# rohitsinghlab/SAME

Measured on AMD Instinct MI355X. Metric: cell-pairs/sec on 100k×100k cost build + edge-cross sweep; % HBM roofline, higher is better.
Workload: dtype f64

## Files before the change

### include/same_hip_diag.h

```cpp
#ifndef SAME_HIP_DIAG_H
#define SAME_HIP_DIAG_H

#include "same_hip.h"

#ifdef __cplusplus
extern "C" {
#endif

enum { SAME_STAT_LAUNCHES = 0, SAME_STAT_FILLS = 1, SAME_STAT_COPIES = 2, SAME_STAT_WAITS = 3, SAME_STAT_GREEDY_READBACKS = 4, SAME_STAT_COUNT = 5 };
int same_ctx_stat(same_ctx *ctx, int which, int64_t *out);


int same_timer_start(same_ctx *ctx);
int same_timer_stop(same_ctx *ctx, float *out_ms);
int same_timer_mark(same_ctx *ctx);
int same_timer_read(same_ctx *ctx, float *out_ms);

int same_ctx_pci_bus_id(same_ctx *ctx, char *out, size_t out_len);
int same_dev_mem_info(same_ctx *ctx, int64_t *out_free, int64_t *out_total);

#define SAME_SPREAD_INFO_LEN 14
int same_dev_alloc_spread(same_ctx *ctx, size_t bytes, void **out_dptr, int64_t *out_info);

#define SAME_Q32_MAX_TYPES 32
int same_quantize_u32_dev(same_ctx *ctx, const double *dsrc, int64_t n, double offset, double scale,
                          uint32_t *ddst);
int same_dense_cost_q32_dev(same_ctx *ctx, const uint32_t *dAq, const uint32_t *dRq, const double *dA,
                            const double *dR, int T, const double *daxy, const double *drxy, int64_t n_r,
                            int64_t row_begin, int64_t row_end, double w, double inv_scale,
                            double rel_tol, double *dout, int64_t ld);

int same_comm_gather_time(same_ctx *ctx, float *out_ms, int64_t *out_send_bytes);

#ifdef __cplusplus
}
#endif
#endif
```

### same_amd/_lib.py

```python
import ctypes
import os
import sys
import threading

import numpy as np

_HERE = os.path.dirname(os.path.abspath(__file__))
LIB_PATH = os.environ.get("SAME_HIP_LIB") or os.path.join(_HERE, "libsame_hip.so")

c_i64 = ctypes.c_int64
c_int = ctypes.c_int
c_dbl = ctypes.c_double
c_flt = ctypes.c_float
c_vp = ctypes.c_void_p
c_sz = ctypes.c_size_t

UNIQUE_ID_BYTES = 128
ABI_VERSION = 8
DT_U8, DT_I32, DT_U64, DT_F64 = 0, 1, 2, 3
OP_SUM, OP_MAX, OP_MIN = 0, 1, 2
SPREAD_INFO_LEN = 14
MAX_KNN = 448
MAX_TYPES = 4096

_PROTOTYPES = {
    "same_abi_version": [],
    "same_device_count": [ctypes.POINTER(c_int)],
    "same_ctx_create": [c_int, ctypes.POINTER(c_vp)],
    "same_ctx_destroy": [c_vp],
    "same_ctx_sync": [c_vp],
    "same_strerror": [c_int],
    "same_last_error": [c_vp],
    "same_ctx_info": [c_vp, ctypes.c_char_p, c_sz, ctypes.POINTER(c_int), ctypes.POINTER(c_i64)],
    "same_ctx_pci_bus_id": [c_vp, ctypes.c_char_p, c_sz],
    "same_ctx_stat": [c_vp, c_int, ctypes.POINTER(c_i64)],
    "same_dev_alloc": [c_vp, c_sz, ctypes.POINTER(c_vp)],
    "same_dev_free": [c_vp, c_vp],
    "same_dev_alloc_spread": [c_vp, c_sz, ctypes.POINTER(c_vp), ctypes.POINTER(c_i64)],
    "same_h2d": [c_vp, c_vp, c_vp, c_sz],
    "same_d2h": [c_vp, c_vp, c_vp, c_sz],
    "same_dev_memset": [c_vp, c_vp, c_int, c_sz],
    "same_d2d": [c_vp, c_vp, c_vp, c_sz],
    "same_dev_mem_info": [c_vp, ctypes.POINTER(c_i64), ctypes.POINTER(c_i64)],
    "same_ctx_release_scratch": [c_vp],
    "same_timer_start": [c_vp],
    "same_timer_stop": [c_vp, ctypes.POINTER(c_flt)],
    "same_timer_mark": [c_vp],
    "same_timer_read": [c_vp, ctypes.POINTER(c_flt)],
    "same_pair_cost_f64": [c_vp, c_vp, c_vp, c_i64, c_i64, c_int, c_vp, c_vp, c_vp, c_i64, c_dbl, c_vp],
    "same_pair_cost_f32": [c_vp, c_vp, c_vp, c_i64, c_i64, c_int, c_vp, c_vp, c_vp, c_i64, c_flt, c_vp],
    "same_dense_cost_f64_dev": [c_vp, c_vp, c_vp, c_int, c_vp, c_vp, c_i64, c_i64, c_i64, c_dbl, c_vp, c_i64],
    "same_dense_cost_f32_dev": [c_vp, c_vp, c_vp, c_int, c_vp, c_vp, c_i64, c_i64, c_i64, c_flt, c_vp, c_i64],
    "same_dense_cost_f64": [c_vp, c_vp, c_vp, c_i64, c_i64, c_int, c_vp, c_vp, c_i64, c_i64, c_dbl, c_vp, c_i64],
    "same_dense_cost_f32": [c_vp, c_vp, c_vp, c_i64, c_i64, c_int, c_vp, c_vp, c_i64, c_i64, c_flt, c_vp, c_i64],
    "same_quantize_u32_dev": [c_vp, c_vp, c_i64, c_dbl, c_dbl, c_vp],
    "same_dense_cost_q32_dev": [c_vp, c_vp, c_vp, c_vp, c_vp, c_int, c_vp, c_vp, c_i64, c_i64, c_i64, c_dbl, c_dbl, c_dbl, c_vp, c_i64],
    "same_knn_prune": [c_vp, c_vp, c_i64, c_vp, c_i64, c_i64, c_i64, c_dbl, c_int, c_vp, c_vp, c_vp],
    "same_knn_prune_dev": [c_vp, c_vp, c_vp, c_i64, c_i64, c_i64, c_dbl, c_int, c_vp, c_vp, c_vp],
    "same_knn_index_build": [c_vp, c_vp, c_i64, c_dbl, ctypes.POINTER(c_vp)],
    "same_knn_index_destroy": [c_vp],
    "same_knn_prune_indexed_dev": [c_vp, c_vp, c_vp, c_i64, c_i64, c_int, c_vp, c_vp, c_vp],
    "same_padded_cost_f64_dev": [c_vp, c_vp, c_vp, c_int, c_vp, c_vp, c_i64, c_i64, c_int, c_vp, c_dbl, c_vp],
    "same_padded_cost_f32_dev": [c_vp, c_vp, c_vp, c_int, c_vp, c_vp, c_i64, c_i64, c_int, c_vp, c_flt, c_vp],
    "same_tri_classify": [c_vp, c_vp, c_i64, c_vp, c_i64, c_dbl, c_int, c_dbl, c_vp, c_vp, c_vp, c_vp],
    "same_tri_sign_weight": [c_vp, c_vp, c_vp, c_i64, c_vp, c_i64, c_vp, c_vp],
    "same_sweep_bind": [c_vp, c_vp, c_i64, c_vp, c_vp, c_i64, c_i64, c_vp, c_i64, ctypes.POINTER(c_vp)],
    "same_sweep_unbind": [c_vp],
    "same_orient_sweep": [c_vp, c_vp, c_i64, ctypes.POINTER(c_i64), c_vp, ctypes.POINTER(c_i64), c_vp],
    "same_orient_sweep_x": [c_vp, c_vp, c_i64, ctypes.POINTER(c_i64), c_vp, ctypes.POINTER(c_i64), c_vp, c_vp, c_vp],
    "same_xyorder_sweep": [c_vp, c_vp, c_i64, c_vp, c_i64, c_vp, c_i64, c_vp, c_vp, c_vp, c_vp, c_vp],
    "same_area_flip": [c_vp, c_vp, c_i64, c_vp, c_i64, c_vp, c_i64, c_vp, c_vp, c_vp, c_vp, c_vp],
    "same_tri_classify_dev": [c_vp, c_vp, c_vp, c_i64, c_dbl, c_int, c_dbl, c_vp, c_vp, c_vp, c_vp],
    "same_tri_sign_weight_dev": [c_vp, c_vp, c_vp, c_vp, c_i64, c_vp, c_vp],
    "same_area_flip_dev": [c_vp, c_vp, c_vp, c_vp, c_i64, c_vp, c_vp, c_vp, c_vp, c_vp],
    "same_xyorder_sweep_dev": [c_vp, c_vp, c_i64, c_vp, c_vp, c_i64, c_vp, c_vp, c_vp, c_vp, c_vp],
    "same_orient_sweep_dev": [c_vp, c_vp, ctypes.POINTER(c_i64), c_vp, ctypes.POINTER(c_i64)],
    "same_orient_flags_dev": [c_vp, c_vp, c_i64, c_i64, c_vp],
    "same_orient_from_flags_dev": [c_vp, c_vp, ctypes.POINTER(c_i64), c_vp, ctypes.POINTER(c_i64)],
    "same_first_candidate_dev": [c_vp, c_vp, c_i64, c_int, c_vp],
    "same_pair_rowmin": [c_vp, c_vp, c_vp, c_i64, c_i64, c_vp],
    "same_assign_matrix": [c_vp, c_vp, c_vp, c_i64, c_vp, c_i64, c_i64, c_dbl, c_vp],
    "same_greedy_match": [c_vp, c_vp, c_vp, c_i64, c_i64, c_i64, c_vp, c_vp, ctypes.POINTER(c_int)],
    "same_tri_flip_stats": [c_vp, c_vp, c_vp, c_vp, c_i64, c_vp, c_vp, c_i64, c_vp, c_vp, c_vp],
    "same_collapse_candidates": [c_vp, c_vp, c_i64, c_vp, c_i64, c_int, c_dbl, c_int, c_dbl, c_vp, c_vp, c_dbl, c_vp, c_vp, c_vp],
    "same_greedy_disjoint": [c_vp, c_vp, c_vp, c_i64, c_i64, c_vp, ctypes.POINTER(c_int)],
    "same_batched_assign": [c_vp, c_i64, c_vp, c_vp, c_vp, c_vp, c_vp],
    "same_eager_signs": [c_vp, c_vp, c_i64, c_vp, c_i64, c_vp, c_i64, c_int, c_vp],
    "same_window_count": [c_vp, c_vp, c_i64, c_vp, c_i64, c_vp, c_vp],
    "same_section_create": [c_vp, c_vp, c_vp, c_int, c_vp, c_vp, c_i64, c_int, ctypes.POINTER(c_vp)],
# ... 277 lines not shown
```

### same_amd/csrc/common.h

```cpp
#pragma once
#include <hip/hip_runtime.h>

#include <cstdint>
#include <cstdio>
#include <cstring>
#include <string>
#include <vector>

#include "same_hip_diag.h"

struct ncclComm;

enum Slot {
    SL_A = 0, SL_R, SL_AXY, SL_RXY, SL_PAIRS, SL_OUT0, SL_OUT1, SL_OUT2, SL_TRIS, SL_MATCH,
    SL_SIGN, SL_SIZE, SL_TYPE, SL_FLAG0, SL_FLAG1, SL_FLAG2, SL_COUNTS, SL_X, SL_MASK,
    SL_K_HIST, SL_K_RANK, SL_K_SXY, SL_K_SIDX, SL_K_BBOX, SL_K_START,
    SL_COUNT
};

struct same_spread_alloc {
    char *va = nullptr;
    size_t bytes = 0;
    std::vector<void *> handles;
};
void same_spread_release(same_spread_alloc &a);

struct same_ctx {
    int device = -1;
    hipStream_t stream = nullptr;
    hipStream_t comm_stream = nullptr;
    hipEvent_t ev0 = nullptr, ev1 = nullptr;
    hipEvent_t ev_ready = nullptr, ev_gathered = nullptr;
    hipEvent_t ev_gather0 = nullptr;
    bool gather_open = false, gather_stamped = false, in_group = false;
    size_t gather_bytes = 0;
    void *slot[SL_COUNT] = {};
    size_t slot_bytes[SL_COUNT] = {};
    void *pinned = nullptr;
    size_t pinned_bytes = 0;
    std::string err;
    int cu_count = 0;
    ncclComm *comm = nullptr;
    int nranks = 1, rank = 0;
    std::vector<same_spread_alloc> spread;
    int64_t stats[SAME_STAT_COUNT] = {};
};

#define SAME_LAUNCH(ctx, kernel, grid, block, lds, ...)                                  \
    do {                                                                                 \
        ++(ctx)->stats[SAME_STAT_LAUNCHES];                                              \
        hipLaunchKernelGGL(kernel, grid, block, lds, (ctx)->stream, __VA_ARGS__);        \
    } while (0)
#define SAME_FILL(ctx, ptr, value, bytes)                                                \
    do {                                                                                 \
        ++(ctx)->stats[SAME_STAT_FILLS];                                                 \
        HIP_TRY((ctx), hipMemsetAsync((ptr), (value), (bytes), (ctx)->stream));          \
    } while (0)
#define SAME_COPY(ctx, dst, src, bytes, kind)                                            \
    do {                                                                                 \
        ++(ctx)->stats[SAME_STAT_COPIES];                                                \
        HIP_TRY((ctx), hipMemcpyAsync((dst), (src), (bytes), (kind), (ctx)->stream));    \
    } while (0)
#define SAME_WAIT(ctx)                                                                   \
    do {                                                                                 \
        ++(ctx)->stats[SAME_STAT_WAITS];                                                 \
        HIP_TRY((ctx), hipStreamSynchronize((ctx)->stream));                             \
    } while (0)

struct same_sweep {
    same_ctx *ctx = nullptr;
    int64_t Tr = 0, n_r = 0, n_m = 0, P = 0;
    int32_t *tris = nullptr;
    int8_t *sign = nullptr;
    double *rxy = nullptr;
    int32_t *pairs = nullptr;
    int32_t *match = nullptr, *pidx = nullptr;
    uint8_t *flag = nullptr;
    unsigned long long *scan_base = nullptr;
// ... 111 lines not shown
```

### same_amd/csrc/delaunay_dev.hip

```cpp
#include "qhull_margin.h"
#include "window_internal.h"

namespace {

using namespace devmath;
using namespace win;
using scan::Pair;

constexpr int NB_CAP = 128;
constexpr int OWN_CAP = 32;
constexpr int SURV_CAP = 1024;
constexpr int SCAN_CELLS_CAP = 256;
constexpr double SIGN_MARGIN = 1e-12;
constexpr double SCREEN_SLACK = 1e-9;

enum { ST_STATUS = 0, ST_TRIS = 1, ST_WORDS = 8 };

struct Par {
    double x0, y0, cw, r2s, delta, w, sc_m;
    qm::Scale sc;
    double ox[8], oy[8];
    int nx, ny, ncell, n_oct;
};

struct Job {
    const double *xy;
    int64_t n, ncell_cap, cap_out;
    unsigned long long *st;
    unsigned long long *scan_cells, *scan_own;
    unsigned *cell_cnt, *cell_start, *slot, *own_cnt;
    int32_t *cell_of, *sorted, *own_tris, *out;
    Par *par;
};

struct Settings {
    double radius, cos_thr, guard;
};

__device__ __forceinline__ void refuse(const Job &j, unsigned bits) { atomicOr(&j.st[ST_STATUS], (unsigned long long)bits); }
__device__ __forceinline__ unsigned long long status_of(const Job &j) {
    return __hip_atomic_load(&j.st[ST_STATUS], __ATOMIC_RELAXED, __HIP_MEMORY_SCOPE_AGENT);
}
__device__ __forceinline__ int cell_x(const Par &p, double x) {
    const double f = std::floor((x - p.x0) / p.cw);
    return !(f >= 0.0) ? 0 : (f >= (double)p.nx ? p.nx - 1 : (int)f);
}
__device__ __forceinline__ int cell_y(const Par &p, double y) {
    const double f = std::floor((y - p.y0) / p.cw);
    return !(f >= 0.0) ? 0 : (f >= (double)p.ny ? p.ny - 1 : (int)f);
}

__device__ __forceinline__ double block_min(double v, double *sh) {
#pragma unroll
    for (int off = 32; off > 0; off >>= 1) v = fmin(v, __shfl_xor(v, off, 64));
    __syncthreads();
    if ((threadIdx.x & 63) == 0) sh[threadIdx.x >> 6] = v;
    __syncthreads();
    return fmin(fmin(sh[0], sh[1]), fmin(sh[2], sh[3]));
}
__device__ __forceinline__ void block_argmax(double &v, int64_t &i, double *shv, int64_t *shi) {
#pragma unroll
    for (int off = 32; off > 0; off >>= 1) {
        const double ov = __shfl_xor(v, off, 64);
        const int64_t oi = __shfl_xor(i, off, 64);
// ... 183 lines not shown
            while (h >= lo && cross3(sx[hull[h - 2]], sy[hull[h - 2]], sx[hull[h - 1]], sy[hull[h - 1]], sx[a], sy[a]) <= 0.0) --h;
            hull[h++] = a;
        }
        n_hull = h - 1;
        if (n_hull < 3) verdict = 1;
    }
    __syncthreads();
    const int h = n_hull;
    if (!verdict) {
        for (int t = threadIdx.x; t < h; t += blockDim.x) {
            const int a = hull[(t + h - 1) % h], c = hull[t], d = hull[(t + 1) % h];
            const double area2 = std::fabs(cross3(sx[a], sy[a], sx[c], sy[c], sx[d], sy[d]));
            const double chord = std::sqrt((sx[d] - sx[a]) * (sx[d] - sx[a]) + (sy[d] - sy[a]) * (sy[d] - sy[a]));
            if (!(qm::plain_ratio(area2, chord, p.sc) > set.guard)) atomicOr(&verdict, 1);
        }
        for (int64_t q = threadIdx.x; q < (int64_t)k * h; q += blockDim.x) {
            const int s = (int)(q / h), e = (int)(q % h);
            const int a = hull[e], c = hull[(e + 1) % h];
            if (s == a || s == c) continue;
            const double area2 = std::fabs(cross3(sx[a], sy[a], sx[c], sy[c], sx[s], sy[s]));
            const double edge = std::sqrt((sx[c] - sx[a]) * (sx[c] - sx[a]) + (sy[c] - sy[a]) * (sy[c] - sy[a]));
            if (!(qm::plain_ratio(area2, edge, p.sc) > set.guard)) atomicOr(&verdict, 1);
        }
    }
    __syncthreads();
    if (threadIdx.x == 0 && verdict) refuse(j, SAME_DD_IN_DOUBT);
}

__device__ __forceinline__ double max_corner_cos(double2_t a, double2_t b, double2_t c) {
    const double c1 = corner_cos(b, a, c), c2 = corner_cos(a, b, c), c3 = corner_cos(a, c, b);
    return fmax(fmax(c1, c2), c3);
}

__global__ __launch_bounds__(256) void dd_candidate_kernel(Batch<Job> b, Settings set) {
    const Job &j = b.w[blockIdx.y];
    const int64_t pi = (int64_t)blockIdx.x * blockDim.x + threadIdx.x;
    if (pi >= j.n || j.n < 3 || status_of(j)) return;
    const Par &p = *j.par;
    const double *__restrict__ xy = j.xy;
    const int32_t *__restrict__ sorted = j.sorted;
    const unsigned *__restrict__ start = j.cell_start;
    const double2_t P = ld2(xy, pi);
    const int c0 = j.cell_of[pi], cx = c0 % p.nx, cy = c0 / p.nx;
    int32_t nb[NB_CAP];
    int k = 0;
    for (int yy = cy - 1; yy <= cy + 1; ++yy) {
        if (yy < 0 || yy >= p.ny) continue;
        for (int xx = cx - 1; xx <= cx + 1; ++xx) {
            if (xx < 0 || xx >= p.nx) continue;
            const int c = yy * p.nx + xx;
            for (unsigned q = start[c]; q < start[c + 1]; ++q) {
                const int32_t s = sorted[q];
                if (s <= pi) continue;
                const double2_t S = ld2(xy, s);
                const double dx = S.x - P.x, dy = S.y - P.y;
                if (dx * dx + dy * dy >= p.r2s) continue;
                if (k == NB_CAP) { refuse(j, SAME_DD_OVERFLOW); return; }
                nb[k++] = s;
            }
        }
    }
    for (int a = 1; a < k; ++a) {
        const int32_t v = nb[a];
        int q = a - 1;
        while (q >= 0 && nb[q] > v) { nb[q + 1] = nb[q]; --q; }
        nb[q + 1] = v;
    }
    int32_t *own = j.own_tris + pi * (int64_t)OWN_CAP * 3;
    unsigned count = 0;
    for (int a = 0; a < k; ++a) {
        const double2_t Q = ld2(xy, nb[a]);
        for (int bq = a + 1; bq < k; ++bq) {
            const double2_t R = ld2(xy, nb[bq]);
            const double qx = R.x - Q.x, qy = R.y - Q.y;
            if (qx * qx + qy * qy >= p.r2s) continue;
            if (!(max_corner_cos(P, Q, R) < set.cos_thr + SCREEN_SLACK)) continue;
            double2_t B = Q, C = R;
            int32_t ib = nb[a], ic = nb[bq];
            const double o = cross3(P.x, P.y, Q.x, Q.y, R.x, R.y);
            if (o < 0.0) { B = R; C = Q; ib = nb[bq]; ic = nb[a]; }
            const double dx = B.x - P.x, dy = B.y - P.y, ex = C.x - P.x, ey = C.y - P.y;
            const double bl = dx * dx + dy * dy, cl = ex * ex + ey * ey, d = dx * ey - dy * ex;
            if (!(d > 0.0)) { refuse(j, SAME_DD_IN_DOUBT); return; }
            const double ucx = (ey * bl - dy * cl) * 0.5 / d, ucy = (dx * cl - ex * bl) * 0.5 / d;
            const double ccx = P.x + ucx, ccy = P.y + ucy, rad = std::sqrt(ucx * ucx + ucy * ucy);
            const double jd = qm::judge(P.x, P.y, dx, dy, ex, ey, p.sc);
            const double reach = 2.0 * set.guard / (rad * d * jd) + 1e-9 * rad + 1e-12 * (std::fabs(ccx) + std::fabs(ccy));
            const int x_lo = cell_x(p, ccx - (rad + reach)), x_hi = cell_x(p, ccx + (rad + reach));
            const int y_lo = cell_y(p, ccy - (rad + reach)), y_hi = cell_y(p, ccy + (rad + reach));
            if (!(reach < 1e300) || (int64_t)(x_hi - x_lo + 1) * (y_hi - y_lo + 1) > SCAN_CELLS_CAP) { refuse(j, SAME_DD_OVERFLOW); return; }
            bool inside = false, doubt = false;
            for (int yy = y_lo; yy <= y_hi && !inside; ++yy) {
                for (int xx = x_lo; xx <= x_hi && !inside; ++xx) {
                    const int c = yy * p.nx + xx;
                    for (unsigned q = start[c]; q < start[c + 1]; ++q) {
                        const int32_t s = sorted[q];
                        if (s == pi || s == ib || s == ic) continue;
                        const double2_t S = ld2(xy, s);
                        const double ax_ = P.x - S.x, ay_ = P.y - S.y, bx_ = B.x - S.x, by_ = B.y - S.y, fx = C.x - S.x, fy = C.y - S.y;
                        const double ap = ax_ * ax_ + ay_ * ay_, bp = bx_ * bx_ + by_ * by_, cp = fx * fx + fy * fy;
                        const double det = ax_ * (by_ * cp - bp * fy) - ay_ * (bx_ * cp - bp * fx) + ap * (bx_ * fy - by_ * fx);
                        const double perm = (std::fabs(by_ * cp) + std::fabs(bp * fy)) * std::fabs(ax_) +
                                            (std::fabs(bx_ * cp) + std::fabs(bp * fx)) * std::fabs(ay_) +
                                            (std::fabs(bx_ * fy) + std::fabs(by_ * fx)) * ap;
                        if (!(std::fabs(det) > SIGN_MARGIN * perm) || !(std::fabs(det) * jd > set.guard)) {
                            doubt = true;
                            continue;
                        }
                        if (det > 0.0) { inside = true; break; }
                    }
                }
            }
            if (inside) continue;
            if (doubt) { refuse(j, SAME_DD_IN_DOUBT); return; }
            if (count == OWN_CAP) { refuse(j, SAME_DD_OVERFLOW); return; }
            own[3 * count] = (int32_t)pi;
            own[3 * count + 1] = ib;
            own[3 * count + 2] = ic;
            ++count;
        }
    }
    j.own_cnt[pi] = count;
}

__global__ __launch_bounds__(scan::NT) void dd_emit_kernel(Batch<Job> b) {
    __shared__ scan::Shared sh;
    const Job &j = b.w[blockIdx.y];
    if (j.n < 3) return;
    const int64_t n = j.n;
    const int nb = (int)scan::blocks_for(n);
    if ((int)blockIdx.x >= nb) return;
    const unsigned *cnt = j.own_cnt;
    auto val = [&](int64_t i) { return Pair{i < n ? cnt[i] : 0u, 0u}; };
    Pair through;
    const Pair off = scan::exclusive(j.scan_own, (int)blockIdx.x, val, sh, &through);
    const int64_t i = (int64_t)blockIdx.x * scan::NT + threadIdx.x;
    if (i < n) {
        const unsigned c = cnt[i];
        if (c > (unsigned)OWN_CAP || (int64_t)off.a + c > j.cap_out) {
            refuse(j, SAME_DD_OVERFLOW);
        } else {
            const int32_t *src = j.own_tris + i * (int64_t)OWN_CAP * 3;
            int32_t *dst = j.out + 3 * (int64_t)off.a;
            for (unsigned q = 0; q < 3 * c; ++q) dst[q] = src[q];
        }
    }
    if ((int)blockIdx.x == nb - 1 && threadIdx.x == 0) j.st[ST_TRIS] = through.a;
}

struct Layout {
    size_t o_st, o_scan_cells, o_cell_cnt, o_own_cnt, o_scan_own, zero_bytes, o_par, o_cell_start, o_cell_of, o_slot, o_sorted, o_own, total;
    int64_t ncell_cap;
};
Layout layout_for(int64_t n) {
    Layout l{};
    l.ncell_cap = 2 * n + 64;
    Carver cv;
    l.o_st = cv.take(ST_WORDS * 8);
    l.o_scan_cells = cv.take(scan::status_bytes(l.ncell_cap));
    l.o_cell_cnt = cv.take((size_t)l.ncell_cap * 4);
    l.o_own_cnt = cv.take((size_t)n * 4);
    l.o_scan_own = cv.take(scan::status_bytes(n));
    l.zero_bytes = cv.off;
    l.o_par = cv.take(sizeof(Par));
    l.o_cell_start = cv.take((size_t)(l.ncell_cap + 1) * 4);
    l.o_cell_of = cv.take((size_t)n * 4);
    l.o_slot = cv.take((size_t)n * 4);
    l.o_sorted = cv.take((size_t)n * 4);
    l.o_own = cv.take((size_t)n * OWN_CAP * 12);
    l.total = cv.off;
    return l;
}
Job job_on(char *base, const Layout &l, const double *xy, int64_t n, int32_t *out, int64_t cap_out) {
    Job j{};
    j.xy = xy;
    j.n = n;
    j.ncell_cap = l.ncell_cap;
    j.cap_out = cap_out;
    j.st = reinterpret_cast<unsigned long long *>(base + l.o_st);
    j.scan_cells = scan::arg(reinterpret_cast<unsigned long long *>(base + l.o_scan_cells));
    j.cell_cnt = reinterpret_cast<unsigned *>(base + l.o_cell_cnt);
    j.own_cnt = reinterpret_cast<unsigned *>(base + l.o_own_cnt);
    j.scan_own = scan::arg(reinterpret_cast<unsigned long long *>(base + l.o_scan_own));
    j.par = reinterpret_cast<Par *>(base + l.o_par);
    j.cell_start = reinterpret_cast<unsigned *>(base + l.o_cell_start);
    j.cell_of = reinterpret_cast<int32_t *>(base + l.o_cell_of);
    j.slot = reinterpret_cast<unsigned *>(base + l.o_slot);
    j.sorted = reinterpret_cast<int32_t *>(base + l.o_sorted);
    j.own_tris = reinterpret_cast<int32_t *>(base + l.o_own);
    j.out = out;
    return j;
}

int launch_group(same_ctx *ctx, const Job *jobs, int n_j, Settings set) {
    Batch<Job> b{};
    int64_t max_n = 0, max_cells = 0;
    for (int q = 0; q < n_j; ++q) {
        b.w[q] = jobs[q];
        max_n = std::max(max_n, jobs[q].n);
        max_cells = std::max(max_cells, jobs[q].ncell_cap);
    }
    const unsigned nw = (unsigned)n_j;
    SAME_LAUNCH(ctx, dd_setup_kernel, dim3(1, nw), dim3(256), 0, b, set);
    SAME_LAUNCH(ctx, dd_count_kernel, dim3(grid_for(max_n), nw), dim3(256), 0, b);
    SAME_LAUNCH(ctx, dd_cell_scan_kernel, dim3(scan::blocks_for(max_cells), nw), dim3(scan::NT), 0, b);
    SAME_LAUNCH(ctx, dd_scatter_kernel, dim3(grid_for(max_n), nw), dim3(256), 0, b);
    SAME_LAUNCH(ctx, dd_cell_sort_kernel, dim3(grid_for(max_cells), nw), dim3(256), 0, b);
    SAME_LAUNCH(ctx, dd_hull_kernel, dim3(1, nw), dim3(256), 0, b, set);
    SAME_LAUNCH(ctx, dd_candidate_kernel, dim3(grid_for(max_n), nw), dim3(256), 0, b, set);
    SAME_LAUNCH(ctx, dd_emit_kernel, dim3(scan::blocks_for(max_n), nw), dim3(scan::NT), 0, b);
    HIP_TRY(ctx, hipGetLastError());
    return SAME_OK;
}

bool settings_answerable(double radius, int angle_enabled, double cos_thr) {
    return radius > 0.0 && std::isfinite(radius) && angle_enabled && cos_thr == cos_thr && cos_thr < 0.9999;
}

}

extern "C" {

int same_window_delaunay(same_window *const *windows, int n_windows, double radius, int angle_enabled, double cos_thr, double guard,
                         int32_t *out_status, int64_t *out_n_tris) {
    same_ctx *ctx = nullptr;
    SAME_TRY(check_batch(windows, n_windows, &ctx));
    REQUIRE(ctx, out_status && out_n_tris && guard >= 0.0);
    for (int i = 0; i < n_windows; ++i) REQUIRE(ctx, windows[i]->staged == 2 && windows[i]->n_ua < ((int64_t)1 << 30));
    SAME_TRY(same_use(ctx));
    const bool ok = settings_answerable(radius, angle_enabled, cos_thr);
    const Settings set{radius, cos_thr, guard};
    std::vector<Job> jobs;
    std::vector<int> at((size_t)n_windows, -1);
    for (int i = 0; i < n_windows; ++i) {
        same_window *w = windows[i];
        w->dd_ok = 0;
        w->n_dd = 0;
        out_status[i] = !ok ? SAME_DD_NO_ANGLE : (w->n_ua < 3 ? SAME_DD_FEW_POINTS : 0);
        out_n_tris[i] = 0;
        if (out_status[i]) continue;
        const int64_t n = w->n_ua, cap_out = 2 * n;
        const Layout l = layout_for(n);
        SAME_TRY(ensure(ctx, w->dd_work, l.total));
        SAME_TRY(ensure(ctx, w->dd_tris, (size_t)cap_out * 12));
        at[(size_t)i] = (int)jobs.size();
        jobs.push_back(job_on(static_cast<char *>(w->dd_work.p), l, w->axy_c, n, static_cast<int32_t *>(w->dd_tris.p), cap_out));
        jobs.back().ncell_cap = l.ncell_cap;
    }
    if (jobs.empty()) return SAME_OK;
    int rc = SAME_OK;
    for (size_t g = 0; g < jobs.size() && rc == SAME_OK; g += SAME_LAUNCH_WINDOWS) {
        const int n_g = (int)std::min<size_t>(SAME_LAUNCH_WINDOWS, jobs.size() - g);
        ZeroArgs zr[SAME_LAUNCH_WINDOWS];
        for (int q = 0; q < n_g; ++q) {
            const Job &jb = jobs[g + (size_t)q];
            zr[q] = ZeroArgs{{jb.st, nullptr}, {layout_for(jb.n).zero_bytes, 0}};
        }
        rc = launch_zero(ctx, zr, n_g);
        if (rc == SAME_OK) rc = launch_group(ctx, jobs.data() + g, n_g, set);
    }
    unsigned long long *h = static_cast<unsigned long long *>(ctx->pinned);
    for (size_t q = 0; q < jobs.size() && rc == SAME_OK; ++q) {
        hipError_t e = hipMemcpyAsync(h + 2 * q, jobs[q].st, 16, hipMemcpyDeviceToHost, ctx->stream);
        ++ctx->stats[SAME_STAT_COPIES];
        if (e != hipSuccess) rc = same_fail(ctx, SAME_EIO, "device triangulation status", e);
    }
    if (rc != SAME_OK) {
        (void)hipStreamSynchronize(ctx->stream);
        return rc;
    }
    SAME_WAIT(ctx);
    for (int i = 0; i < n_windows; ++i) {
        if (at[(size_t)i] < 0) continue;
        const unsigned long long *s = h + 2 * at[(size_t)i];
        same_window *w = windows[i];
        out_status[i] = (int32_t)(s[0] & 0x7fffffffu);
        if (out_status[i] == 0) {
            w->n_dd = (int64_t)s[1];
            w->dd_ok = 1;
            out_n_tris[i] = w->n_dd;
        }
    }
    return SAME_OK;
}

int same_delaunay_filtered(same_ctx *ctx, const double *xy, int64_t n, double radius, int angle_enabled, double cos_thr, double guard,
                           int32_t *out_tris, int64_t cap, int64_t *out_n_tris, int32_t *out_status) {
    if (!ctx) return SAME_EINVAL;
    REQUIRE(ctx, (xy || n == 0) && out_n_tris && out_status && n >= 0 && n < ((int64_t)1 << 30) && cap >= 0 && (out_tris || cap == 0) &&
                     guard >= 0.0);
    *out_n_tris = 0;
    *out_status = !settings_answerable(radius, angle_enabled, cos_thr) ? SAME_DD_NO_ANGLE : (n < 3 ? SAME_DD_FEW_POINTS : 0);
    if (*out_status) return SAME_OK;
    SAME_TRY(same_use(ctx));
    const Layout l = layout_for(n);
    double *dxy = nullptr;
    char *work = nullptr;
    int32_t *dout = nullptr;
    SAME_TRY(up_as(ctx, SL_AXY, xy, (size_t)n * 2, &dxy));
    SAME_TRY(slot_as(ctx, SL_X, l.total, &work));
    SAME_TRY(slot_as(ctx, SL_TRIS, (size_t)(2 * n) * 3, &dout));
    Job jb = job_on(work, l, dxy, n, dout, 2 * n);
    SAME_FILL(ctx, work, 0, l.zero_bytes);
    SAME_TRY(launch_group(ctx, &jb, 1, Settings{radius, cos_thr, guard}));
    unsigned long long *h = static_cast<unsigned long long *>(ctx->pinned);
    SAME_COPY(ctx, h, jb.st, 16, hipMemcpyDeviceToHost);
    SAME_WAIT(ctx);
    *out_status = (int32_t)(h[0] & 0x7fffffffu);
    if (*out_status) return SAME_OK;
    const int64_t count = (int64_t)h[1];
    if (count > cap) return SAME_EINVAL;
    if (count) {
        SAME_COPY(ctx, out_tris, dout, (size_t)count * 12, hipMemcpyDeviceToHost);
        SAME_WAIT(ctx);
    }
    *out_n_tris = count;
    return SAME_OK;
}

}
```

Baseline: 615.2 billion.

## Split Delaunay candidate search into list-based multi-kernel pipeline with group-parallel incircle

Result: no change. 614.7 billion, median of 6 (-0.1%).

```diff
diff --git a/include/same_hip_diag.h b/include/same_hip_diag.h
--- a/include/same_hip_diag.h
+++ b/include/same_hip_diag.h
@@ -30,6 +30,9 @@
                             int64_t row_begin, int64_t row_end, double w, double inv_scale,
                             double rel_tol, double *dout, int64_t ld);
 
+int same_dd_set_per_owner(same_ctx *ctx, int on);
+int same_dd_fallbacks(same_ctx *ctx, int64_t *out);
+
 int same_comm_gather_time(same_ctx *ctx, float *out_ms, int64_t *out_send_bytes);
 
 #ifdef __cplusplus
diff --git a/same_amd/_lib.py b/same_amd/_lib.py
--- a/same_amd/_lib.py
+++ b/same_amd/_lib.py
@@ -55,6 +55,8 @@
     "same_dense_cost_f32": [c_vp, c_vp, c_vp, c_i64, c_i64, c_int, c_vp, c_vp, c_i64, c_i64, c_flt, c_vp, c_i64],
     "same_quantize_u32_dev": [c_vp, c_vp, c_i64, c_dbl, c_dbl, c_vp],
     "same_dense_cost_q32_dev": [c_vp, c_vp, c_vp, c_vp, c_vp, c_int, c_vp, c_vp, c_i64, c_i64, c_i64, c_dbl, c_dbl, c_dbl, c_vp, c_i64],
+    "same_dd_set_per_owner": [c_vp, c_int],
+    "same_dd_fallbacks": [c_vp, ctypes.POINTER(c_i64)],
     "same_knn_prune": [c_vp, c_vp, c_i64, c_vp, c_i64, c_i64, c_i64, c_dbl, c_int, c_vp, c_vp, c_vp],
     "same_knn_prune_dev": [c_vp, c_vp, c_vp, c_i64, c_i64, c_i64, c_dbl, c_int, c_vp, c_vp, c_vp],
     "same_knn_index_build": [c_vp, c_vp, c_i64, c_dbl, ctypes.POINTER(c_vp)],
diff --git a/same_amd/csrc/common.h b/same_amd/csrc/common.h
--- a/same_amd/csrc/common.h
+++ b/same_amd/csrc/common.h
@@ -44,6 +44,8 @@
     int nranks = 1, rank = 0;
     std::vector<same_spread_alloc> spread;
     int64_t stats[SAME_STAT_COUNT] = {};
+    int dd_per_owner = 0;
+    int64_t dd_fallbacks = 0;
 };
 
 #define SAME_LAUNCH(ctx, kernel, grid, block, lds, ...)                                  \
diff --git a/same_amd/csrc/delaunay_dev.hip b/same_amd/csrc/delaunay_dev.hip
--- a/same_amd/csrc/delaunay_dev.hip
+++ b/same_amd/csrc/delaunay_dev.hip
@@ -13,8 +13,14 @@
 constexpr int SCAN_CELLS_CAP = 256;
 constexpr double SIGN_MARGIN = 1e-12;
 constexpr double SCREEN_SLACK = 1e-9;
-
-enum { ST_STATUS = 0, ST_TRIS = 1, ST_WORDS = 8 };
+constexpr int64_t LIST_PER_POINT = 64;
+constexpr int64_t LIST_N_MAX = 0x7FFFFFFF / (NB_CAP * (NB_CAP - 1) / 2);
+constexpr int SG = 16;
+constexpr int IG = 16;
+constexpr unsigned IC_BLOCKS = 2048;
+
+enum { ST_STATUS = 0, ST_TRIS = 1, ST_CANDS = 2, ST_FALLBACK = 3, ST_BACK = 4, ST_WORDS = 8 };
+enum : uint8_t { V_PENDING = 0, V_KEEP = 1, V_DROP = 2, V_DOUBT = 3, V_OVERFLOW = 4 };
 
 struct Par {
     double x0, y0, cw, r2s, delta, w, sc_m;
@@ -23,13 +29,22 @@
     int nx, ny, ncell, n_oct;
 };
 
+struct Cand {
+    int32_t p, ib, ic, c0;
+    unsigned wh;
+    double jd;
+};
+
 struct Job {
     const double *xy;
-    int64_t n, ncell_cap, cap_out;
+    int64_t n, ncell_cap, cap_out, cap_cand;
+    int per_owner;
     unsigned long long *st;
-    unsigned long long *scan_cells, *scan_own;
-    unsigned *cell_cnt, *cell_start, *slot, *own_cnt;
-    int32_t *cell_of, *sorted, *own_tris, *out;
+    unsigned long long *scan_cells, *scan_own, *scan_scr;
+    unsigned *cell_cnt, *cell_start, *slot, *own_cnt, *nb_cnt, *scr_cnt, *scr_off;
+    int32_t *cell_of, *sorted, *own_tris, *out, *nb;
+    Cand *cand;
+    uint8_t *verdict;
     Par *par;
 };
 
@@ -279,10 +294,258 @@
     return fmax(fmax(c1, c2), c3);
 }
 
-__global__ __launch_bounds__(256) void dd_candidate_kernel(Batch<Job> b, Settings set) {
+__device__ __forceinline__ bool screened(const Par &p, const Settings &set, double2_t P, double2_t Q, double2_t R) {
+    const double qx = R.x - Q.x, qy = R.y - Q.y;
+    if (qx * qx + qy * qy >= p.r2s) return false;
+    return max_corner_cos(P, Q, R) < set.cos_thr + SCREEN_SLACK;
+}
+
+enum { CC_OK = 0, CC_DOUBT = 1, CC_OVERFLOW = 2 };
+struct Circle {
+    int32_t ib, ic;
+    int x_lo, x_hi, y_lo, y_hi;
+    double jd;
+    double2_t B, C;
+};
+__device__ __forceinline__ int circle_of(const Par &p, const Settings &set, double2_t P, double2_t Q, double2_t R, int32_t iq, int32_t ir,
+                                         Circle &o) {
+    o = Circle{};
+    o.B = Q; o.C = R; o.ib = iq; o.ic = ir;
+    const double ori = cross3(P.x, P.y, Q.x, Q.y, R.x, R.y);
+    if (ori < 0.0) { o.B = R; o.C = Q; o.ib = ir; o.ic = iq; }
+    const double dx = o.B.x - P.x, dy = o.B.y - P.y, ex = o.C.x - P.x, ey = o.C.y - P.y;
+    const double bl = dx * dx + dy * dy, cl = ex * ex + ey * ey, d = dx * ey - dy * ex;
+    if (!(d > 0.0)) return CC_DOUBT;
+    const double ucx = (ey * bl - dy * cl) * 0.5 / d, ucy = (dx * cl - ex * bl) * 0.5 / d;
+    const double ccx = P.x + ucx, ccy = P.y + ucy, rad = std::sqrt(ucx * ucx + ucy * ucy);
+    o.jd = qm::judge(P.x, P.y, dx, dy, ex, ey, p.sc);
+    const double reach = 2.0 * set.guard / (rad * d * o.jd) + 1e-9 * rad + 1e-12 * (std::fabs(ccx) + std::fabs(ccy));
+    o.x_lo = cell_x(p, ccx - (rad + reach)); o.x_hi = cell_x(p, ccx + (rad + reach));
+    o.y_lo = cell_y(p, ccy - (rad + reach)); o.y_hi = cell_y(p, ccy + (rad + reach));
+    if (!(reach < 1e300) || (int64_t)(o.x_hi - o.x_lo + 1) * (o.y_hi - o.y_lo + 1) > SCAN_CELLS_CAP) return CC_OVERFLOW;
+    return CC_OK;
+}
+
+enum { IC_OUTSIDE = 0, IC_INSIDE = 1, IC_DOUBT = 2 };
+__device__ __forceinline__ int incircle(double2_t P, double2_t B, double2_t C, double2_t S, double jd, double guard) {
+    const double ax_ = P.x - S.x, ay_ = P.y - S.y, bx_ = B.x - S.x, by_ = B.y - S.y, fx = C.x - S.x, fy = C.y - S.y;
+    const double ap = ax_ * ax_ + ay_ * ay_, bp = bx_ * bx_ + by_ * by_, cp = fx * fx + fy * fy;
+    const double det = ax_ * (by_ * cp - bp * fy) - ay_ * (bx_ * cp - bp * fx) + ap * (bx_ * fy - by_ * fx);
+    const double perm = (std::fabs(by_ * cp) + std::fabs(bp * fy)) * std::fabs(ax_) +
+                        (std::fabs(bx_ * cp) + std::fabs(bp * fx)) * std::fabs(ay_) +
+                        (std::fabs(bx_ * fy) + std::fabs(by_ * fx)) * ap;
+    if (!(std::fabs(det) > SIGN_MARGIN * perm) || !(std::fabs(det) * jd > guard)) return IC_DOUBT;
+    return det > 0.0 ? IC_INSIDE : IC_OUTSIDE;
+}
+
+
+__global__ __launch_bounds__(256) void dd_nb_kernel(Batch<Job> b) {
+    const Job &j = b.w[blockIdx.y];
+    const int64_t pi = (int64_t)blockIdx.x * blockDim.x + threadIdx.x;
+    if (pi >= j.n || j.n < 3 || j.per_owner || status_of(j)) return;
+    const Par &p = *j.par;
+    const double *__restrict__ xy = j.xy;
+    const int32_t *__restrict__ sorted = j.sorted;
+    const unsigned *__restrict__ start = j.cell_start;
+    const double2_t P = ld2(xy, pi);
+    const int c0 = j.cell_of[pi], cx = c0 % p.nx, cy = c0 / p.nx;
+    unsigned cur[9], end[9];
+    int32_t head[9];
+#pragma unroll
+    for (int t = 0; t < 9; ++t) {
+        const int yy = cy - 1 + t / 3, xx = cx - 1 + t % 3;
+        cur[t] = end[t] = 0;
+        if (yy >= 0 && yy < p.ny && xx >= 0 && xx < p.nx) { cur[t] = start[yy * p.nx + xx]; end[t] = start[yy * p.nx + xx + 1]; }
+        head[t] = INT32_MAX;
+        for (; cur[t] < end[t]; ++cur[t]) {
+            const int32_t s = sorted[cur[t]];
+            if (s > pi) { head[t] = s; break; }
+        }
+    }
+    int32_t *nb = j.nb + pi * (int64_t)NB_CAP;
+    int k = 0;
+    for (;;) {
+        int32_t s = INT32_MAX;
+        int at = -1;
+#pragma unroll
+        for (int t = 0; t < 9; ++t)
+            if (head[t] < s) { s = head[t]; at = t; }
+        if (at < 0) break;
+#pragma unroll
+        for (int t = 0; t < 9; ++t)
+            if (t == at) { ++cur[t]; head[t] = cur[t] < end[t] ? sorted[cur[t]] : INT32_MAX; }
+        const double2_t S = ld2(xy, s);
+        const double dx = S.x - P.x, dy = S.y - P.y;
+        if (dx * dx + dy * dy >= p.r2s) continue;
+        if (k == NB_CAP) { refuse(j, SAME_DD_OVERFLOW); return; }
+        nb[k++] = s;
+    }
+    j.nb_cnt[pi] = (unsigned)k;
+}
+
+__device__ __forceinline__ void next_pair(int k, int step, int &a, int &bq) {
+    bq += step;
+    while (bq >= k && a < k - 1) { ++a; bq = bq - k + a + 1; }
+}
+__global__ __launch_bounds__(256) void dd_screen_count_kernel(Batch<Job> b, Settings set) {
+    const Job &j = b.w[blockIdx.y];
+    const int64_t o = ((int64_t)blockIdx.x * blockDim.x + threadIdx.x) / SG;
+    const int l = (int)(threadIdx.x % SG);
+    if (o >= j.n || j.n < 3 || j.per_owner || status_of(j)) return;
+    const Par &p = *j.par;
+    const double *__restrict__ xy = j.xy;
+    const int k = (int)min(j.nb_cnt[o], (unsigned)NB_CAP);
+    const int32_t *nb = j.nb + o * NB_CAP;
+    const double2_t P = ld2(xy, o);
+    const unsigned long long gmask = ((1ull << SG) - 1) << ((threadIdx.x & 63) & ~(unsigned)(SG - 1));
+    const int pairs = k * (k - 1) / 2;
+    int a = 0, bq = 1;
+    next_pair(k, l, a, bq);
+    unsigned total = 0;
+    for (int t0 = 0; t0 < pairs; t0 += SG) {
+        const bool ok = t0 + l < pairs && screened(p, set, P, ld2(xy, nb[a]), ld2(xy, nb[bq]));
+        total += (unsigned)__popcll(__ballot(ok) & gmask);
+        next_pair(k, SG, a, bq);
+    }
+    if (l == 0) j.scr_cnt[o] = total;
+}
+
+__global__ __launch_bounds__(scan::NT) void dd_owner_scan_kernel(Batch<Job> b) {
+    __shared__ scan::Shared sh;
+    const Job &j = b.w[blockIdx.y];
+    if (j.n < 3 || j.per_owner || status_of(j)) return;
+    const int64_t n = j.n;
+    const int nb = (int)scan::blocks_for(n);
+    if ((int)blockIdx.x >= nb) return;
+    const unsigned *cnt = j.scr_cnt;
+    auto val = [&](int64_t i) { return Pair{i < n ? cnt[i] : 0u, 0u}; };
+    Pair through;
+    const Pair off = scan::exclusive(j.scan_scr, (int)blockIdx.x, val, sh, &through);
+    const int64_t i = (int64_t)blockIdx.x * scan::NT + threadIdx.x;
+    if (i < n) j.scr_off[i] = off.a;
+    if ((int)blockIdx.x == nb - 1 && threadIdx.x == 0) {
+        j.st[ST_CANDS] = through.a;
+        if ((int64_t)through.a > j.cap_cand) j.st[ST_FALLBACK] = 1;
+    }
+}
+
+__global__ __launch_bounds__(256) void dd_screen_write_kernel(Batch<Job> b, Settings set) {
+    const Job &j = b.w[blockIdx.y];
+    const int64_t o = ((int64_t)blockIdx.x * blockDim.x + threadIdx.x) / SG;
+    const int l = (int)(threadIdx.x % SG);
+    if (o >= j.n || j.n < 3 || j.per_owner || status_of(j) || j.st[ST_FALLBACK]) return;
+    const Par &p = *j.par;
+    const double *__restrict__ xy = j.xy;
+    const int k = (int)min(j.nb_cnt[o], (unsigned)NB_CAP);
+    const int32_t *nb = j.nb + o * NB_CAP;
+    const double2_t P = ld2(xy, o);
+    const unsigned lane = threadIdx.x & 63;
+    const unsigned long long gmask = ((1ull << SG) - 1) << (lane & ~(unsigned)(SG - 1)), below = gmask & ((1ull << lane) - 1);
+    const int pairs = k * (k - 1) / 2;
+    int a = 0, bq = 1;
+    next_pair(k, l, a, bq);
+    int64_t at = j.scr_off[o];
+    for (int t0 = 0; t0 < pairs; t0 += SG) {
+        const int32_t iq = t0 + l < pairs ? nb[a] : 0, ir = t0 + l < pairs ? nb[bq] : 0;
+        const double2_t Q = ld2(xy, iq), R = ld2(xy, ir);
+        const bool ok = t0 + l < pairs && screened(p, set, P, Q, R);
+        const unsigned long long m = __ballot(ok) & gmask;
+        if (ok) {
+            const int64_t c = at + __popcll(m & below);
+            Circle cc;
+            const int r = circle_of(p, set, P, Q, R, iq, ir, cc);
+            if (c >= 0 && c < j.cap_cand) {
+                Cand &cd = j.cand[c];
+                cd.p = (int32_t)o;
+                cd.ib = cc.ib;
+                cd.ic = cc.ic;
+                cd.c0 = r == CC_OK ? cc.y_lo * p.nx + cc.x_lo : 0;
+                cd.wh = r == CC_OK ? (unsigned)(cc.x_hi - cc.x_lo + 1) | (unsigned)(cc.y_hi - cc.y_lo + 1) << 16 : 0u;
+                cd.jd = cc.jd;
+                j.verdict[c] = r == CC_OK ? V_PENDING : (r == CC_DOUBT ? V_DOUBT : V_OVERFLOW);
+            }
+        }
+        at += __popcll(m);
+        next_pair(k, SG, a, bq);
+    }
+}
+
+__global__ __launch_bounds__(256) void dd_incircle_kernel(Batch<Job> b, Settings set) {
+    const Job &j = b.w[blockIdx.y];
+    if (j.n < 3 || j.per_owner || status_of(j) || j.st[ST_FALLBACK]) return;
+    const int64_t total = (int64_t)j.st[ST_CANDS];
+    const Par &p = *j.par;
+    const double *__restrict__ xy = j.xy;
+    const int32_t *__restrict__ sorted = j.sorted;
+    const unsigned *__restrict__ start = j.cell_start;
+    const int l = (int)(threadIdx.x % IG);
+    const unsigned long long gmask = ((1ull << IG) - 1) << ((threadIdx.x & 63) & ~(unsigned)(IG - 1));
+    const int64_t stride = (int64_t)gridDim.x * (blockDim.x / IG);
+    for (int64_t c = ((int64_t)blockIdx.x * blockDim.x + threadIdx.x) / IG; c < total; c += stride) {
+        if (j.verdict[c] != V_PENDING) continue;
+        const Cand cd = j.cand[c];
+        const int64_t wx = cd.wh & 0xFFFFu, wy = cd.wh >> 16;
+        if (cd.p < 0 || cd.p >= j.n || cd.ib < 0 || cd.ib >= j.n || cd.ic < 0 || cd.ic >= j.n || wx < 1 || wy < 1 || cd.c0 < 0 ||
+            cd.c0 + (wy - 1) * p.nx + wx > p.ncell) {
+            if (l == 0) j.verdict[c] = V_OVERFLOW;
+            continue;
+        }
+        const double2_t P = ld2(xy, cd.p), B = ld2(xy, cd.ib), C = ld2(xy, cd.ic);
+        unsigned tot = 0;
+        for (int64_t r = 0; r < wy; ++r) tot += start[cd.c0 + r * p.nx + wx] - start[cd.c0 + r * p.nx];
+        int64_t row = 0;
+        unsigned lo = start[cd.c0], len = start[cd.c0 + wx] - lo, cum = 0;
+        bool inside = false, doubt = false;
+        for (unsigned f0 = 0; f0 < tot; f0 += IG) {
+            const unsigned f = f0 + (unsigned)l;
+            if (f < tot) {
+                while (f >= cum + len) {
+                    cum += len;
+                    ++row;
+                    lo = start[cd.c0 + row * p.nx];
+                    len = start[cd.c0 + row * p.nx + wx] - lo;
+                }
+                const int32_t s = sorted[lo + (f - cum)];
+                if (s != cd.p && s != cd.ib && s != cd.ic) {
+                    const int v = incircle(P, B, C, ld2(xy, s), cd.jd, set.guard);
+                    inside |= v == IC_INSIDE;
+                    doubt |= v == IC_DOUBT;
+                }
+            }
+            if (__ballot(inside) & gmask) break;
+        }
+        const bool any_in = (__ballot(inside) & gmask) != 0, any_doubt = (__ballot(doubt) & gmask) != 0;
+        if (l == 0) j.verdict[c] = any_in ? V_DROP : (any_doubt ? V_DOUBT : V_KEEP);
+    }
+}
+
+__global__ __launch_bounds__(256) void dd_walk_kernel(Batch<Job> b) {
+    const Job &j = b.w[blockIdx.y];
+    const int64_t pi = (int64_t)blockIdx.x * blockDim.x + threadIdx.x;
+    if (pi >= j.n || j.n < 3 || j.per_owner || status_of(j) || j.st[ST_FALLBACK]) return;
+    const int64_t lo = j.scr_off[pi], hi = lo + j.scr_cnt[pi];
+    if (hi > j.cap_cand) { refuse(j, SAME_DD_OVERFLOW); return; }
+    int32_t *own = j.own_tris + pi * (int64_t)OWN_CAP * 3;
+    unsigned count = 0;
+    for (int64_t c = lo; c < hi; ++c) {
+        const uint8_t v = j.verdict[c];
+        if (v == V_DROP) continue;
+        if (v == V_DOUBT) { refuse(j, SAME_DD_IN_DOUBT); return; }
+        if (v != V_KEEP) { refuse(j, SAME_DD_OVERFLOW); return; }
+        if (count == OWN_CAP) { refuse(j, SAME_DD_OVERFLOW); return; }
+        own[3 * count] = (int32_t)pi;
+        own[3 * count + 1] = j.cand[c].ib;
+        own[3 * count + 2] = j.cand[c].ic;
+        ++count;
+    }
+    j.own_cnt[pi] = count;
+}
+
+__global__ __launch_bounds__(256) void dd_per_owner_kernel(Batch<Job> b, Settings set) {
     const Job &j = b.w[blockIdx.y];
     const int64_t pi = (int64_t)blockIdx.x * blockDim.x + threadIdx.x;
     if (pi >= j.n || j.n < 3 || status_of(j)) return;
+    if (!j.per_owner && !j.st[ST_FALLBACK]) return;
     const Par &p = *j.par;
     const double *__restrict__ xy = j.xy;
     const int32_t *__restrict__ sorted = j.sorted;
@@ -319,42 +582,21 @@
         const double2_t Q = ld2(xy, nb[a]);
         for (int bq = a + 1; bq < k; ++bq) {
             const double2_t R = ld2(xy, nb[bq]);
-            const double qx = R.x - Q.x, qy = R.y - Q.y;
-            if (qx * qx + qy * qy >= p.r2s) continue;
-            if (!(max_corner_cos(P, Q, R) < set.cos_thr + SCREEN_SLACK)) continue;
-            double2_t B = Q, C = R;
-            int32_t ib = nb[a], ic = nb[bq];
-            const double o = cross3(P.x, P.y, Q.x, Q.y, R.x, R.y);
-            if (o < 0.0) { B = R; C = Q; ib = nb[bq]; ic = nb[a]; }
-            const double dx = B.x - P.x, dy = B.y - P.y, ex = C.x - P.x, ey = C.y - P.y;
-            const double bl = dx * dx + dy * dy, cl = ex * ex + ey * ey, d = dx * ey - dy * ex;
-            if (!(d > 0.0)) { refuse(j, SAME_DD_IN_DOUBT); return; }
-            const double ucx = (ey * bl - dy * cl) * 0.5 / d, ucy = (dx * cl - ex * bl) * 0.5 / d;
-            const double ccx = P.x + ucx, ccy = P.y + ucy, rad = std::sqrt(ucx * ucx + ucy * ucy);
-            const double jd = qm::judge(P.x, P.y, dx, dy, ex, ey, p.sc);
-            const double reach = 2.0 * set.guard / (rad * d * jd) + 1e-9 * rad + 1e-12 * (std::fabs(ccx) + std::fabs(ccy));
-            const int x_lo = cell_x(p, ccx - (rad + reach)), x_hi = cell_x(p, ccx + (rad + reach));
-            const int y_lo = cell_y(p, ccy - (rad + reach)), y_hi = cell_y(p, ccy + (rad + reach));
-            if (!(reach < 1e300) || (int64_t)(x_hi - x_lo + 1) * (y_hi - y_lo + 1) > SCAN_CELLS_CAP) { refuse(j, SAME_DD_OVERFLOW); return; }
+            if (!screened(p, set, P, Q, R)) continue;
+            Circle cc;
+            const int r = circle_of(p, set, P, Q, R, nb[a], nb[bq], cc);
+            if (r == CC_DOUBT) { refuse(j, SAME_DD_IN_DOUBT); return; }
+            if (r == CC_OVERFLOW) { refuse(j, SAME_DD_OVERFLOW); return; }
             bool inside = false, doubt = false;
-            for (int yy = y_lo; yy <= y_hi && !inside; ++yy) {
-                for (int xx = x_lo; xx <= x_hi && !inside; ++xx) {
+            for (int yy = cc.y_lo; yy <= cc.y_hi && !inside; ++yy) {
+                for (int xx = cc.x_lo; xx <= cc.x_hi && !inside; ++xx) {
                     const int c = yy * p.nx + xx;
                     for (unsigned q = start[c]; q < start[c + 1]; ++q) {
                         const int32_t s = sorted[q];
-                        if (s == pi || s == ib || s == ic) continue;
-                        const double2_t S = ld2(xy, s);
-                        const double ax_ = P.x - S.x, ay_ = P.y - S.y, bx_ = B.x - S.x, by_ = B.y - S.y, fx = C.x - S.x, fy = C.y - S.y;
-                        const double ap = ax_ * ax_ + ay_ * ay_, bp = bx_ * bx_ + by_ * by_, cp = fx * fx + fy * fy;
-                        const double det = ax_ * (by_ * cp - bp * fy) - ay_ * (bx_ * cp - bp * fx) + ap * (bx_ * fy - by_ * fx);
-                        const double perm = (std::fabs(by_ * cp) + std::fabs(bp * fy)) * std::fabs(ax_) +
-                                            (std::fabs(bx_ * cp) + std::fabs(bp * fx)) * std::fabs(ay_) +
-                                            (std::fabs(bx_ * fy) + std::fabs(by_ * fx)) * ap;
-                        if (!(std::fabs(det) > SIGN_MARGIN * perm) || !(std::fabs(det) * jd > set.guard)) {
-                            doubt = true;
-                            continue;
-                        }
-                        if (det > 0.0) { inside = true; break; }
+                        if (s == pi || s == cc.ib || s == cc.ic) continue;
+                        const int v = incircle(P, cc.B, cc.C, ld2(xy, s), cc.jd, set.guard);
+                        if (v == IC_DOUBT) { doubt = true; continue; }
+                        if (v == IC_INSIDE) { inside = true; break; }
                     }
                 }
             }
@@ -362,8 +604,8 @@
             if (doubt) { refuse(j, SAME_DD_IN_DOUBT); return; }
             if (count == OWN_CAP) { refuse(j, SAME_DD_OVERFLOW); return; }
             own[3 * count] = (int32_t)pi;
-            own[3 * count + 1] = ib;
-            own[3 * count + 2] = ic;
+            own[3 * count + 1] = cc.ib;
+            own[3 * count + 2] = cc.ic;
             ++count;
         }
     }
@@ -396,18 +638,23 @@
 }
 
 struct Layout {
-    size_t o_st, o_scan_cells, o_cell_cnt, o_own_cnt, o_scan_own, zero_bytes, o_par, o_cell_start, o_cell_of, o_slot, o_sorted, o_own, total;
-    int64_t ncell_cap;
+    size_t o_st, o_scan_cells, o_cell_cnt, o_own_cnt, o_scan_own, o_scan_scr, zero_bytes, o_par, o_cell_start, o_cell_of, o_slot, o_sorted,
+        o_own, o_nb_cnt, o_scr_cnt, o_scr_off, o_nb, o_cand, o_verdict, total;
+    int64_t ncell_cap, cap_cand;
 };
 Layout layout_for(int64_t n) {
     Layout l{};
     l.ncell_cap = 2 * n + 64;
+    const bool list = n <= LIST_N_MAX;
+    const int64_t nl = list ? n : 0;
+    l.cap_cand = LIST_PER_POINT * nl;
     Carver cv;
     l.o_st = cv.take(ST_WORDS * 8);
     l.o_scan_cells = cv.take(scan::status_bytes(l.ncell_cap));
     l.o_cell_cnt = cv.take((size_t)l.ncell_cap * 4);
     l.o_own_cnt = cv.take((size_t)n * 4);
     l.o_scan_own = cv.take(scan::status_bytes(n));
+    l.o_scan_scr = cv.take(scan::status_bytes(nl));
     l.zero_bytes = cv.off;
     l.o_par = cv.take(sizeof(Par));
     l.o_cell_start = cv.take((size_t)(l.ncell_cap + 1) * 4);
@@ -415,15 +662,23 @@
     l.o_slot = cv.take((size_t)n * 4);
     l.o_sorted = cv.take((size_t)n * 4);
     l.o_own = cv.take((size_t)n * OWN_CAP * 12);
+    l.o_nb_cnt = cv.take((size_t)nl * 4);
+    l.o_scr_cnt = cv.take((size_t)nl * 4);
+    l.o_scr_off = cv.take((size_t)nl * 4);
+    l.o_nb = cv.take((size_t)nl * NB_CAP * 4);
+    l.o_cand = cv.take((size_t)l.cap_cand * sizeof(Cand));
+    l.o_verdict = cv.take((size_t)l.cap_cand);
     l.total = cv.off;
     return l;
 }
-Job job_on(char *base, const Layout &l, const double *xy, int64_t n, int32_t *out, int64_t cap_out) {
+Job job_on(char *base, const Layout &l, const double *xy, int64_t n, int32_t *out, int64_t cap_out, bool per_owner) {
     Job j{};
     j.xy = xy;
     j.n = n;
     j.ncell_cap = l.ncell_cap;
     j.cap_out = cap_out;
+    j.cap_cand = l.cap_cand;
+    j.per_owner = per_owner || n > LIST_N_MAX;
     j.st = reinterpret_cast<unsigned long long *>(base + l.o_st);
     j.scan_cells = scan::arg(reinterpret_cast<unsigned long long *>(base + l.o_scan_cells));
     j.cell_cnt = reinterpret_cast<unsigned *>(base + l.o_cell_cnt);
@@ -435,17 +690,28 @@
     j.slot = reinterpret_cast<unsigned *>(base + l.o_slot);
     j.sorted = reinterpret_cast<int32_t *>(base + l.o_sorted);
     j.own_tris = reinterpret_cast<int32_t *>(base + l.o_own);
+    j.scan_scr = scan::arg(reinterpret_cast<unsigned long long *>(base + l.o_scan_scr));
+    j.nb_cnt = reinterpret_cast<unsigned *>(base + l.o_nb_cnt);
+    j.scr_cnt = reinterpret_cast<unsigned *>(base + l.o_scr_cnt);
+    j.scr_off = reinterpret_cast<unsigned *>(base + l.o_scr_off);
+    j.nb = reinterpret_cast<int32_t *>(base + l.o_nb);
+    j.cand = reinterpret_cast<Cand *>(base + l.o_cand);
+    j.verdict = reinterpret_cast<uint8_t *>(base + l.o_verdict);
     j.out = out;
     return j;
 }
 
 int launch_group(same_ctx *ctx, const Job *jobs, int n_j, Settings set) {
     Batch<Job> b{};
-    int64_t max_n = 0, max_cells = 0;
+    int64_t max_n = 0, max_cells = 0, max_list_n = 0, max_cand = 0;
     for (int q = 0; q < n_j; ++q) {
         b.w[q] = jobs[q];
         max_n = std::max(max_n, jobs[q].n);
         max_cells = std::max(max_cells, jobs[q].ncell_cap);
+        if (!jobs[q].per_owner) {
+            max_list_n = std::max(max_list_n, jobs[q].n);
+            max_cand = std::max(max_cand, jobs[q].cap_cand);
+        }
     }
     const unsigned nw = (unsigned)n_j;
     SAME_LAUNCH(ctx, dd_setup_kernel, dim3(1, nw), dim3(256), 0, b, set);
@@ -454,7 +720,16 @@
     SAME_LAUNCH(ctx, dd_scatter_kernel, dim3(grid_for(max_n), nw), dim3(256), 0, b);
     SAME_LAUNCH(ctx, dd_cell_sort_kernel, dim3(grid_for(max_cells), nw), dim3(256), 0, b);
     SAME_LAUNCH(ctx, dd_hull_kernel, dim3(1, nw), dim3(256), 0, b, set);
-    SAME_LAUNCH(ctx, dd_candidate_kernel, dim3(grid_for(max_n), nw), dim3(256), 0, b, set);
+    if (max_list_n > 0) {
+        SAME_LAUNCH(ctx, dd_nb_kernel, dim3(grid_for(max_list_n), nw), dim3(256), 0, b);
+        SAME_LAUNCH(ctx, dd_screen_count_kernel, dim3(grid_for(max_list_n * SG), nw), dim3(256), 0, b, set);
+        SAME_LAUNCH(ctx, dd_owner_scan_kernel, dim3(scan::blocks_for(max_list_n), nw), dim3(scan::NT), 0, b);
+        SAME_LAUNCH(ctx, dd_screen_write_kernel, dim3(grid_for(max_list_n * SG), nw), dim3(256), 0, b, set);
+        const unsigned ic_blocks = (unsigned)std::min<int64_t>(IC_BLOCKS, std::max<int64_t>(1, ceil_div(max_cand, 256 / IG)));
+        SAME_LAUNCH(ctx, dd_incircle_kernel, dim3(ic_blocks, nw), dim3(256), 0, b, set);
+        SAME_LAUNCH(ctx, dd_walk_kernel, dim3(grid_for(max_list_n), nw), dim3(256), 0, b);
+    }
+    SAME_LAUNCH(ctx, dd_per_owner_kernel, dim3(grid_for(max_n), nw), dim3(256), 0, b, set);
     SAME_LAUNCH(ctx, dd_emit_kernel, dim3(scan::blocks_for(max_n), nw), dim3(scan::NT), 0, b);
     HIP_TRY(ctx, hipGetLastError());
     return SAME_OK;
@@ -491,7 +766,8 @@
         SAME_TRY(ensure(ctx, w->dd_work, l.total));
         SAME_TRY(ensure(ctx, w->dd_tris, (size_t)cap_out * 12));
         at[(size_t)i] = (int)jobs.size();
-        jobs.push_back(job_on(static_cast<char *>(w->dd_work.p), l, w->axy_c, n, static_cast<int32_t *>(w->dd_tris.p), cap_out));
+        jobs.push_back(job_on(static_cast<char *>(w->dd_work.p), l, w->axy_c, n, static_cast<int32_t *>(w->dd_tris.p), cap_out,
+                              ctx->dd_per_owner != 0));
         jobs.back().ncell_cap = l.ncell_cap;
     }
     if (jobs.empty()) return SAME_OK;
@@ -508,7 +784,7 @@
     }
     unsigned long long *h = static_cast<unsigned long long *>(ctx->pinned);
     for (size_t q = 0; q < jobs.size() && rc == SAME_OK; ++q) {
-        hipError_t e = hipMemcpyAsync(h + 2 * q, jobs[q].st, 16, hipMemcpyDeviceToHost, ctx->stream);
+        hipError_t e = hipMemcpyAsync(h + ST_BACK * q, jobs[q].st, ST_BACK * 8, hipMemcpyDeviceToHost, ctx->stream);
         ++ctx->stats[SAME_STAT_COPIES];
         if (e != hipSuccess) rc = same_fail(ctx, SAME_EIO, "device triangulation status", e);
     }
@@ -519,8 +795,9 @@
     SAME_WAIT(ctx);
     for (int i = 0; i < n_windows; ++i) {
         if (at[(size_t)i] < 0) continue;
-        const unsigned long long *s = h + 2 * at[(size_t)i];
+        const unsigned long long *s = h + ST_BACK * at[(size_t)i];
         same_window *w = windows[i];
+        ctx->dd_fallbacks += s[ST_FALLBACK] != 0;
         out_status[i] = (int32_t)(s[0] & 0x7fffffffu);
         if (out_status[i] == 0) {
             w->n_dd = (int64_t)s[1];
@@ -547,12 +824,13 @@
     SAME_TRY(up_as(ctx, SL_AXY, xy, (size_t)n * 2, &dxy));
     SAME_TRY(slot_as(ctx, SL_X, l.total, &work));
     SAME_TRY(slot_as(ctx, SL_TRIS, (size_t)(2 * n) * 3, &dout));
-    Job jb = job_on(work, l, dxy, n, dout, 2 * n);
+    Job jb = job_on(work, l, dxy, n, dout, 2 * n, ctx->dd_per_owner != 0);
     SAME_FILL(ctx, work, 0, l.zero_bytes);
     SAME_TRY(launch_group(ctx, &jb, 1, Settings{radius, cos_thr, guard}));
     unsigned long long *h = static_cast<unsigned long long *>(ctx->pinned);
-    SAME_COPY(ctx, h, jb.st, 16, hipMemcpyDeviceToHost);
+    SAME_COPY(ctx, h, jb.st, ST_BACK * 8, hipMemcpyDeviceToHost);
     SAME_WAIT(ctx);
+    ctx->dd_fallbacks += h[ST_FALLBACK] != 0;
     *out_status = (int32_t)(h[0] & 0x7fffffffu);
     if (*out_status) return SAME_OK;
     const int64_t count = (int64_t)h[1];
@@ -565,4 +843,18 @@
     return SAME_OK;
 }
 
-}
+int same_dd_set_per_owner(same_ctx *ctx, int on) {
+    if (!ctx) return SAME_EINVAL;
+    REQUIRE(ctx, on == 0 || on == 1);
+    ctx->dd_per_owner = on;
+    return SAME_OK;
+}
+
+int same_dd_fallbacks(same_ctx *ctx, int64_t *out) {
+    if (!ctx) return SAME_EINVAL;
+    REQUIRE(ctx, out);
+    *out = ctx->dd_fallbacks;
+    return SAME_OK;
+}
+
+}
```
